# RemoteSensingTools/vSmartMOM.jl

Hardware: AMD Instinct MI355X
Metric: spectral-points/s (whole node) for rt_run, O2-A band (higher is better)
Workload: dtype f64; 1 GPU; C2: O2-A 759-770 nm, nStokes=3, Nquad=20 (N=60), 40 layers, 10000 spectral points/GPU, m=0..2, Rayleigh+synthetic O2 absorption, Lambertian 0.15; ranks=1, collective_backend=none (1 rank), N=60, layers=40, points_per_gpu=10000, fourier_moments=3

## Files before the change

### include/vsmartmom_hip.h

```cpp
#ifndef VSMARTMOM_HIP_H
#define VSMARTMOM_HIP_H

#include <stddef.h>
#include <stdint.h>

#ifdef __cplusplus
extern "C" {
#endif

typedef enum vsm_status {
  VSM_OK = 0,
  VSM_ERR_INVALID_ARG = 1,
  VSM_ERR_UNSUPPORTED = 2,
  VSM_ERR_HIP = 3,
  VSM_ERR_NO_DEVICE = 4
} vsm_status;

typedef enum vsm_iface {
  VSM_IFACE_00 = 0,
  VSM_IFACE_01 = 1,
  VSM_IFACE_10 = 2,
  VSM_IFACE_11 = 3
} vsm_iface;

// ... 310 lines not shown
                              const vsm_composite_f64* comp, const vsm_added_f64* added_scratch, void* stream);
int vsm_layer_forward_mix_f32(const vsm_quad_f32* q, int S, int m, int ndoubl, const float* dtau, const float* varpi,
                              const float* tau_sum, const float* F0, int ncomp, const float* Zpp_comp, const float* Zmp_comp,
                              const float* fcomp, float* z_scratch, int toa, const vsm_composite_f32* comp,
                              const vsm_added_f32* added_scratch, void* stream);
int vsm_mix_Z_f64(int N, int S, int ncomp, const double* Zpp_comp, const double* Zmp_comp, const double* fcomp, double* Zpp,
                  double* Zmp, void* stream);
int vsm_mix_Z_f32(int N, int S, int ncomp, const float* Zpp_comp, const float* Zmp_comp, const float* fcomp, float* Zpp,
                  float* Zmp, void* stream);
int vsm_mix_Z_moments_f64(int N, int S, int ncomp, int nm, const double* const* Zpp_comp_h, const double* const* Zmp_comp_h, int single,
                          const double* fcomp, double* Zpp, double* Zmp, void* stream);
int vsm_mix_Z_moments_f32(int N, int S, int ncomp, int nm, const float* const* Zpp_comp_h, const float* const* Zmp_comp_h, int single,
                          const float* fcomp, float* Zpp, float* Zmp, void* stream);

typedef struct vsm_run vsm_run;
enum { VSM_RUN_SOURCES_ONLY = 1, VSM_RUN_ZW_TAIL = 2 };
int vsm_run_supported(int N, int n_stokes, int coupling);
size_t vsm_run_workspace_bytes(int N, int n_stokes, int S, int nm, const int* coupling_h);
int vsm_run_supported_f32(int N, int n_stokes, int coupling);
size_t vsm_run_workspace_bytes_f32(int N, int n_stokes, int S, int nm, const int* coupling_h);
int vsm_run_create_f64(const vsm_quad_f64* q, int S, int nm, const int* m_h, const int* coupling_h, void* workspace,
                       size_t workspace_bytes, vsm_run** run);
int vsm_run_create_f32(const vsm_quad_f32* q, int S, int nm, const int* m_h, const int* coupling_h, void* workspace,
                       size_t workspace_bytes, vsm_run** run);
int vsm_run_create_ex_f64(const vsm_quad_f64* q, int S, int nm, const int* m_h, const int* coupling_h, void* workspace,
                          size_t workspace_bytes, unsigned flags, vsm_run** run);
int vsm_run_create_ex_f32(const vsm_quad_f32* q, int S, int nm, const int* m_h, const int* coupling_h, void* workspace,
                          size_t workspace_bytes, unsigned flags, vsm_run** run);
int vsm_run_layer_f64(vsm_run* run, int ndoubl, const double* dtau, const double* varpi, const double* tau_sum,
                      const double* F0, int ncomp, const double* const* Zpp, const double* const* Zmp, long long z_stride,
                      const double* fcomp, int toa, const int* layer_coupling_h, void* stream);
int vsm_run_layer_f32(vsm_run* run, int ndoubl, const float* dtau, const float* varpi, const float* tau_sum,
                      const float* F0, int ncomp, const float* const* Zpp, const float* const* Zmp, long long z_stride,
                      const float* fcomp, int toa, const int* layer_coupling_h, void* stream);
int vsm_run_export_f64(vsm_run* run, const vsm_composite_f64* comps, void* stream);
int vsm_run_export_f32(vsm_run* run, const vsm_composite_f32* comps, void* stream);
int vsm_run_import_f64(vsm_run* run, const vsm_composite_f64* comps, void* stream);
int vsm_run_import_f32(vsm_run* run, const vsm_composite_f32* comps, void* stream);
int vsm_run_zw_tail(vsm_run* run);
int vsm_run_destroy(vsm_run* run);
int vsm_stokes_coupling_f64(int N, int n_stokes, int nblocks, const double* Zpp, const double* Zmp, int* mask_d, void* stream);
int vsm_stokes_coupling_f32(int N, int n_stokes, int nblocks, const float* Zpp, const float* Zmp, int* mask_d, void* stream);

typedef struct vsm_added_rs_f64 {
  double *ier_mp, *iet_pp, *ier_pm, *iet_mm;
  double *ieJ0_p, *ieJ0_m;
  int K;
  int reserved;
} vsm_added_rs_f64;
typedef struct vsm_added_rs_f32 {
  float *ier_mp, *iet_pp, *ier_pm, *iet_mm;
  float *ieJ0_p, *ieJ0_m;
  int K;
  int reserved;
// ... 82 lines not shown
```

### vsmartmom.jl_amd/_lib.py

```python
from __future__ import annotations

import ctypes as C
import os

_HERE = os.path.dirname(os.path.abspath(__file__))
LIB_PATH = os.environ.get("VSM_LIB_PATH") or os.path.join(_HERE, "lib", "libvsmartmom_hip.so")


class VSMError(RuntimeError):
    pass


class vsm_quad_f64(C.Structure):
    _fields_ = [("mu", C.c_void_p), ("wt", C.c_void_p), ("N", C.c_int), ("n_stokes", C.c_int),
                ("i_mu0", C.c_int), ("mu0", C.c_double)]


class vsm_quad_f32(C.Structure):
    _fields_ = [("mu", C.c_void_p), ("wt", C.c_void_p), ("N", C.c_int), ("n_stokes", C.c_int),
                ("i_mu0", C.c_int), ("mu0", C.c_float)]


class vsm_added(C.Structure):
    _fields_ = [("r_mp", C.c_void_p), ("t_pp", C.c_void_p), ("r_pm", C.c_void_p), ("t_mm", C.c_void_p),
# ... 105 lines not shown
    "vsm_elemental_inelastic_rrs_{T}": (_I, [_P, _I, _I, _I, _P, _P, _P, _P, _P, _P]),
    "vsm_doubling_inelastic_rrs_{T}": (_I, [_I, _I, _I, _I, _P, _P, _P, _P, _P, _P]),
    "vsm_interaction_inelastic_rrs_{T}": (_I, [_I, _I, _I, _P, _P, _P, _P, _P, _P, _P]),
    "vsm_copy_added_to_composite_ie_{T}": (_I, [_I, _I, _P, _P, _P]),
    "vsm_postprocess_vza_ie_{T}": (_I, [_I, _I, _I, _I, _I, _P, _P, _P, _P, _P, _P, _P]),
    "vsm_run_supported": (_I, [_I, _I, _I]),
    "vsm_run_workspace_bytes": (_SZ, [_I, _I, _I, _I, _P]),
    "vsm_run_supported_f32": (_I, [_I, _I, _I]),
    "vsm_run_workspace_bytes_f32": (_SZ, [_I, _I, _I, _I, _P]),
    "vsm_run_create_{T}": (_I, [_P, _I, _I, _P, _P, _P, _SZ, _P]),
    "vsm_run_create_ex_{T}": (_I, [_P, _I, _I, _P, _P, _P, _SZ, C.c_uint, _P]),
    "vsm_run_layer_{T}": (_I, [_P, _I, _P, _P, _P, _P, _I, _P, _P, _LL, _P, _I, _P, _P]),
    "vsm_run_export_{T}": (_I, [_P, _P, _P]),
    "vsm_run_import_{T}": (_I, [_P, _P, _P]),
    "vsm_run_zw_tail": (_I, [_P]),
    "vsm_run_destroy": (_I, [_P]),
    "vsm_stokes_coupling_{T}": (_I, [_I, _I, _I, _P, _P, _P, _P]),
    "vsm_level_radiance_work_elems": (_SZ, [_I, _I]),
    "vsm_level_radiance_{T}": (_I, [_I, _I, _I, _I, _P, _P, _P, _P, _P, _LL, _P, _P, _P, _P, _P, _P, _P]),
    "vsm_level_radiance_oplevel_{T}": (_I, [_I, _I, _I, _I, _P, _P, _P, _P, _P, _LL, _P, _P, _P, _P, _P, _P, _P]),
    "vsm_test_lds_mm_{T}": (_I, [_I, _I, _P, _P, _P, _P]),
    "vsm_test_lds_inv_{T}": (_I, [_I, _I, _P, _P, _I, _P, _P]),
    "vsm_test_poison_lds": (_I, [_P]),
}


def exported_symbols():
    out = []
    for name in _SIGS:
        if "{T}" in name:
# ... 90 lines not shown
```

### vsmartmom.jl_amd/core_rt.py

```python
from __future__ import annotations

import ctypes as C
import dataclasses
import math
import os
from dataclasses import dataclass
from typing import List, Optional

import numpy as np
import torch

from . import _lib
from . import host_model as H
from .architectures import GPU, CPU, architecture, array_type, devi, synchronize_if_gpu, to_host

IFACE = {"00": 0, "01": 1, "10": 2, "11": 3}
MOMENT_BATCH = 4
MOMENT_BATCH_MAX = 24
MOMENT_BATCHING = True
THERMAL_FUSION = True
NATIVE_RUN = True
NATIVE_SOURCES_ONLY = True
NATIVE_ZW_TAIL = True
NATIVE_DROPIN = True
REFERENCE_ORDER = False


def _require_gpu(arch):
    if not isinstance(arch, GPU):
        raise _lib.VSMError("vsmartmom.jl_amd provides the MI355X path only; architecture %r has no compute path here "
                            "(no CPU fallback by design)" % (arch,))
    if not torch.cuda.is_available():
        raise _lib.VSMError("no MI355X visible to HIP (torch.cuda.is_available() is False)")
    if arch.device_index != torch.cuda.current_device():
        raise _lib.VSMError("architecture GPU(%d) is not the current HIP device (%d): one process per GPU -- call "
                            "torch.cuda.set_device(%d) first" % (arch.device_index, torch.cuda.current_device(),
                                                                 arch.device_index))

# ... 470 lines not shown

def _native_open(comp: CompositeLayer, dq: DeviceQuad, m: int, mask: int, import_arrays: bool) -> bool:
    L = _lib.lib()
    N, ns, S = comp.N, dq.n_stokes, comp.nSpec
    if not run_supported(comp.dtype, N, ns, mask):
        return False
    marr, carr = (C.c_int * 1)(int(m)), (C.c_int * 1)(int(mask))
    nbytes = run_workspace_bytes(comp.dtype, N, ns, S, 1, carr)
    ws = comp._native_ws
    if ws is None or ws.numel() * 8 < nbytes:
        ws = comp._native_ws = _lib.poison(torch.empty(max(nbytes // 8, 2), dtype=torch.float64, device=comp._arr["R_mp"].device))
    q = dq.cstruct()
    comp._native_q = (q, dq)
    run = C.c_void_p()
    flags = 1 if (comp._sources_only and NATIVE_SOURCES_ONLY) else 0
    _lib.call("vsm_run_create_ex", comp.dtype, C.byref(q), S, 1, marr, carr, _ptr(ws), nbytes, flags, C.byref(run))
    if import_arrays:
        try:
            cc = (_lib.vsm_composite * 1)(comp._cstruct_raw())
            _lib.call("vsm_run_import", comp.dtype, run, cc, _stream_ptr())
        except Exception:
            L.vsm_run_destroy(run)
            raise
    comp._native = NativeSlot(run, int(m), int(mask), stokes_groups(ns, mask))
    return True


def _rt_kernel_native(comp: CompositeLayer, props: DeviceLayerOptics, tau_sum, m: int, dq: DeviceQuad, iz: int, F0, dtau,
                      ndoubl: int) -> bool:
    N, ns, S = comp.N, dq.n_stokes, comp.nSpec
# ... 352 lines not shown
                return set()
        return {i for i, mom in enumerate(self.moments) if run_supported(self.dt, self.N, self.pol.n, int(self.coupling[mom["m"]]))}

    def _run_layers_native(self, group, comps, sources_only: bool = True, export_at=None):
        L = _lib.lib()
        nm, N, S, ns = len(group), self.N, self.S, self.pol.n
        marr = (C.c_int * nm)(*[int(mom["m"]) for mom in group])
        carr = (C.c_int * nm)(*[int(self.coupling[mom["m"]]) for mom in group])
        nbytes = run_workspace_bytes(self.dt, N, ns, S, nm, carr)
        ws = getattr(self, "_native_ws", None)
        if ws is None or ws.numel() * 8 < nbytes:
            ws = self._native_ws = _lib.poison(torch.empty(max(nbytes // 8, 2), dtype=torch.float64, device=self.dev))
        q = self.dq.cstruct()
        run = C.c_void_p()
        flags = 1 if (sources_only and NATIVE_SOURCES_ONLY) else 0
        _lib.call("vsm_run_create_ex", self.dt, C.byref(q), S, nm, marr, carr, _ptr(ws), nbytes, flags, C.byref(run))
        try:
            if NATIVE_ZW_TAIL and not torch.cuda.is_current_stream_capturing():
                _lib.check(L.vsm_run_zw_tail(run))
            for iz in range(self.Nz):
                ly0 = group[0]["layers"][iz]
                props = [mom["layers"][iz]["props"] for mom in group]
                p0 = props[0]
                zpp = (C.c_void_p * nm)(*[p.Zpp.data_ptr() for p in props])
                zmp = (C.c_void_p * nm)(*[p.Zmp.data_ptr() for p in props])
                ncomp = 0 if p0.fcomp is None else int(p0.fcomp.shape[1])
                lc = (C.c_int * nm)(*[self._layer_coupling(mom["m"], iz) for mom in group])
                run_layer_native_(run, nm, int(ly0["nd"]), ly0["dtau"], p0.varpi, ly0["tau_sum"], self.F0, ncomp, zpp, zmp,
                                  0 if ncomp else p0.z_stride, p0.fcomp, iz == 0, lc, self.dt)
                if export_at and (iz + 1) in export_at:
# ... 149 lines not shown
```

### vsmartmom.jl_amd/csrc/vsm_api.hip

```cpp
#include <map>
#include <mutex>
#include <set>
#include <utility>
#include <vector>
#include <stdlib.h>
#include <string.h>

#include "build_id.h"
#include "vsm_internal.h"

namespace vsm {

static thread_local char g_err[512] = "";

void set_error(const char* fmt, ...) {
  va_list ap;
  va_start(ap, fmt);
  vsnprintf(g_err, sizeof(g_err), fmt, ap);
  va_end(ap);
}
int hip_fail(hipError_t e, const char* what) {
  set_error("HIP error %d (%s) in %s", (int)e, hipGetErrorString(e), what);
  return VSM_ERR_HIP;
}
// ... 17 lines not shown
    return slot < o.slot;
  }
};
struct scratch_buf {
  void* ptr = nullptr;
  size_t sz = 0;
};
struct retired_buf {
  int dev;
  void* ptr;
  hipEvent_t ev;
};
std::mutex g_scratch_mu;
std::map<scratch_key, scratch_buf> g_scratch;
std::vector<retired_buf> g_retired;

void reap_retired(int dev, bool wait) {
  for (size_t i = 0; i < g_retired.size();) {
    retired_buf& r = g_retired[i];
    if (r.dev == dev && (wait ? hipEventSynchronize(r.ev) == hipSuccess : hipEventQuery(r.ev) == hipSuccess)) {
      (void)hipEventDestroy(r.ev);
      (void)hipFree(r.ptr);
      g_retired[i] = g_retired.back();
      g_retired.pop_back();
    } else {
      ++i;
    }
  }
}
}
// ... 31 lines not shown
    e = hipEventCreateWithFlags(&ev, hipEventDisableTiming);
    if (e == hipSuccess) e = hipEventRecord(ev, st);
    if (e != hipSuccess) {
      if (ev) (void)hipEventDestroy(ev);
      (void)hipFree(p);
      hip_fail(e, "hipEventRecord(scratch retire)");
      return nullptr;
    }
    g_retired.push_back(retired_buf{dev, b.ptr, ev});
  }
  b.ptr = p;
  b.sz = want;
  return p;
}

int release_scratch() {
  int dev = 0;
  hipError_t e = hipGetDevice(&dev);
  if (e != hipSuccess) return hip_fail(e, "hipGetDevice(release_scratch)");
  if ((e = hipDeviceSynchronize()) != hipSuccess) return hip_fail(e, "hipDeviceSynchronize(release_scratch)");
  std::lock_guard<std::mutex> lk(g_scratch_mu);
  reap_retired(dev, true);
  for (auto it = g_scratch.begin(); it != g_scratch.end();) {
    if (it->first.dev == dev) {
      if (it->second.ptr) (void)hipFree(it->second.ptr);
      it = g_scratch.erase(it);
    } else {
      ++it;
    }
  }
  return VSM_OK;
}

namespace {
std::mutex g_attr_mu;
std::set<std::pair<int, const void*>> g_attr_done;
std::mutex g_cu_mu;
std::map<int, int> g_cu;
}

namespace {
// ... 896 lines not shown
```

### vsmartmom.jl_amd/csrc/vsm_internal.h

```cpp
#pragma once
#include "vsm_common.h"

namespace vsm {

template <typename T>
struct quad {
  const T* mu;
  const T* wt;
  int N;
  int n_stokes;
  int i_mu0;
  T mu0;
};
template <typename T>
struct added {
  T *r_mp, *t_pp, *r_pm, *t_mm, *j0_p, *j0_m;
  long long mat_stride;
  int d_symmetric;
};
template <typename T>
struct composite {
  T *R_mp, *R_pm, *T_pp, *T_mm, *J0_p, *J0_m;
};

// ... 227 lines not shown
template <typename ST>
int strip128_doubling(int N, int n_stokes, int S, int ndoubl, ST* expk, const added<ST>& a, hipStream_t st);
template <typename ST>
int strip128_interaction11(int N, int S, const composite<ST>& c, const added<ST>& a, hipStream_t st);
inline bool strip128_f32_supported(int N) { return N > 96 && N <= 128; }

bool strip128_lin_dbl_supported(int N);
template <typename ST>
int strip128_doubling_lin(int N, int S, int P, int nd, int ns, ST* expk, ST* ekl, const added<ST>& a, const added_lin<ST>& al,
                          hipStream_t st);
template <typename ST>
int strip128_interaction11_lin(int N, int S, const composite<ST>& c, const composite_lin<ST>& cl, const added<ST>& a,
                               const added_lin<ST>& al, hipStream_t st);

void* scratch(size_t bytes, int slot, hipStream_t st);
int* device_status();
int release_scratch();
int ensure_dyn_lds(const void* kern, size_t bytes, const char* what);
int cu_count();

}
```

### vsmartmom.jl_amd/csrc/vsm_native.hip

```cpp
#include <stdlib.h>

#include <vector>

#include "vsm_native_dev.h"
#include "vsm_native_run.h"

#ifndef VSM_NATIVE_PARK_RT
#define VSM_NATIVE_PARK_RT 3
#endif

namespace vsm {

struct nlayer_comps {
  double* c[NSUB_MAX];
};

namespace {

template <int RT, int KS, int KZ = KS>
__device__ __forceinline__ void ned_body(nsmem<RT, (4 * KS + 2 > 16 * RT)>& sm, npos<RT>& p, int n, int gsz, unsigned uvmask, int ndoubl,
                                         const double* __restrict__ img, nstrip<RT>& r_s, nstrip<RT>& t_s, int* status) {
  using G = ngeo<RT>;
  constexpr unsigned dP = 0, dQ = G::AF * 8;
  double* jp = sm.vec[0];
// ... 1412 lines not shown
    bool zero = true;
    for (int a = 0; a < ns; ++a) zero = zero && w[(size_t)node * ns + a] == ST(0);
    if (!zero) break;
    ++z;
  }
  if (z == nq) z = 0;
  for (nat_sub& sb : run->subs) sb.kz = ((nq - z) * sb.gsz + 3) / 4;
  run->flags |= VSM_RUN_ZW_TAIL;
  return VSM_OK;
}

template <typename ST, typename Q>
static int run_create(const Q* q, int S, int nm, const int* m, const int* coupling, void* workspace, size_t workspace_bytes,
                      unsigned flags, vsm_run** run_out) {
  VSM_REQUIRE(q && q->mu && q->wt && run_out && m, "vsm_run_create: null argument");
  VSM_REQUIRE((flags & ~(unsigned)(VSM_RUN_SOURCES_ONLY | VSM_RUN_ZW_TAIL)) == 0, "vsm_run_create_ex: unknown flags 0x%x", flags);
  VSM_REQUIRE(S >= 0 && nm >= 1 && nm <= NSUB_MAX, "vsm_run_create: bad S = %d / nm = %d (at most %d moments per run)", S, nm,
              NSUB_MAX);
  vsm_run* run = new vsm_run;
  run->mu = q->mu;
  run->wt = q->wt;
  run->N = q->N;
  run->ns = q->n_stokes;
  run->i_mu0 = q->i_mu0;
  run->mu0 = (double)q->mu0;
  run->elem_size = (int)sizeof(ST);
  run->S = S;
  run->nm = nm;
  run->flags = sizeof(ST) == 8 ? flags : 0u;
  run->m.assign(m, m + nm);
  size_t total = 0;
  const int rc = plan_subs(sizeof(ST) == 4, q->N, q->n_stokes, nm, m, coupling, run->subs, (size_t)S, total);
  if (rc) {
    delete run;
    return rc;
  }
  if (total * sizeof(ST) > workspace_bytes || (total && !workspace) || ((size_t)workspace & 15)) {
    set_error("vsm_run_create: workspace of %zu bytes (16-byte aligned) required, got %zu", total * sizeof(ST), workspace_bytes);
    delete run;
    return VSM_ERR_INVALID_ARG;
  }
  if (run->flags & VSM_RUN_ZW_TAIL) {
    const int rc2 = zw_tail<ST>(run);
    if (rc2) {
// ... 10 lines not shown
    for (auto& cl : run->classes) {
      const nat_sub& h = run->subs[cl[0]];
      if (h.n == sb.n && h.gsz == sb.gsz && h.uvmask == sb.uvmask && (int)cl.size() < NSUB_MAX) {
        cl.push_back((int)i);
        placed = true;
        break;
      }
    }
    if (!placed) run->classes.push_back(std::vector<int>{(int)i});
  }
  *run_out = run;
  return VSM_OK;
}

template <typename ST>
static int run_layer(vsm_run* run, int ndoubl, const ST* dtau, const ST* varpi, const ST* tau_sum, const ST* F0, int ncomp,
                     const ST* const* Zpp, const ST* const* Zmp, long long z_stride, const ST* fcomp, int toa,
                     const int* layer_coupling, void* stream) {
  VSM_REQUIRE(run && dtau && varpi && tau_sum && F0 && Zpp && Zmp, "vsm_run_layer: null argument");
  VSM_REQUIRE(run->elem_size == (int)sizeof(ST), "vsm_run_layer: the run was created for %d-byte arrays", run->elem_size);
  VSM_REQUIRE(ndoubl >= 0 && ndoubl < 60 && ncomp >= 0 && ncomp <= 4 && (ncomp == 0 || fcomp), "vsm_run_layer: bad ndoubl / component mix");
  ++run->layers;
  if (run->S == 0) return VSM_OK;
  hipStream_t st = as_stream(stream);
  int* status = device_status();
  if (!status) return VSM_ERR_HIP;
  const quad<ST> q = run_quad<ST>(run);
  auto trivial = [&](const nat_sub& sb) {
    if (!layer_coupling || layer_coupling[sb.im] < 0) return false;
    for (int a = 0; a < sb.gsz; ++a)
      for (int b = 0; b < sb.gsz; ++b)
        if ((layer_coupling[sb.im] >> (4 * sb.g[a] + sb.g[b])) & 1) return false;
    return true;
  };
  {
    nguard_args<ST> ga;
    for (int k = 0; k < NSUB_MAX; ++k) {
      const int im = k < run->nm ? k : 0;
      VSM_REQUIRE(Zpp[im] && Zmp[im], "vsm_run_layer: null Z of moment %d", im);
      ga.zp[k] = Zpp[im];
      ga.zm[k] = Zmp[im];
      ga.allowed[k] = 0;
    }
    for (const nat_sub& sb : run->subs) {
      if (trivial(sb)) continue;
      for (int a = 0; a < sb.gsz; ++a)
        for (int b = 0; b < sb.gsz; ++b) ga.allowed[sb.im] |= 1u << (4 * sb.g[a] + sb.g[b]);
    }
    const int nmat = ncomp ? ncomp : (z_stride ? run->S : 1);
    hipLaunchKernelGGL((k_coupling_guard<ST>), dim3(nmat, run->nm), dim3(256), 0, st, run->N, run->ns,
                       ncomp ? (long long)run->N * run->N : z_stride, ga, status);
    VSM_LAUNCH_CHECK("k_coupling_guard");
  }
  if constexpr (sizeof(ST) == 4) {
    return native32_run_layer(run, ndoubl, dtau, varpi, tau_sum, F0, ncomp, Zpp, Zmp, z_stride, fcomp, toa, layer_coupling, status, st);
  } else {
  double* const ws = static_cast<double*>(run->ws);
  const int src = (run->flags & VSM_RUN_SOURCES_ONLY) ? 1 : 0;
  size_t pre_total = 0;
  for (const nat_sub& sb : run->subs)
    if (!trivial(sb)) pre_total += pre_stride_rt(sb.rt) * (size_t)run->S;
  double* pre = nullptr;
  if (pre_total) {
    pre = static_cast<double*>(scratch(pre_total * sizeof(double), 3, st));
    if (!pre) return VSM_ERR_HIP;
  }
  size_t off = 0;
  for (const auto& cl : run->classes) {
    const nat_sub& h = run->subs[cl[0]];
    std::vector<int> act, triv[3];
    for (int i : cl) {
      if (!trivial(run->subs[i])) {
        act.push_back(i);
        run->pure_diag[i] = 0;
      } else if (toa) {
        triv[1].push_back(i);
        run->pure_diag[i] = 1;
      } else {
        triv[run->pure_diag[i] ? 2 : 0].push_back(i);
      }
    }
    for (int mode = 0; mode < 3; ++mode) {
      if (triv[mode].empty()) continue;
      ndiag_args da;
      const int nt = (int)triv[mode].size();
      for (int k = 0; k < NSUB_MAX; ++k) {
        const nat_sub& sb = run->subs[triv[mode][k < nt ? k : 0]];
        da.comp[k] = ws + sb.comp_off;
        da.gsz[k] = sb.gsz;
        da.g0[k] = sb.g[0] | (sb.g[1] << 4) | (sb.g[2] << 8) | (sb.g[3] << 12);
      }
      hipLaunchKernelGGL((k_native_diag_layer<ST>), dim3(run->S, nt), dim3(256), 0, st, q, h.rt, h.n, ldexp(1.0, ndoubl), mode, src,
                         dtau, da);
      VSM_LAUNCH_CHECK("k_native_diag_layer");
    }
    const int nsub = (int)act.size();
    if (!nsub) continue;
    npre_args<ST> pa;
    nlayer_comps lc;
    for (int k = 0; k < NSUB_MAX; ++k) {
      const nat_sub& sb = run->subs[act[k < nsub ? k : 0]];
      pa.s[k].m = sb.m;
      pa.s[k].gsz = sb.gsz;
      for (int a = 0; a < 4; ++a) pa.s[k].g[a] = sb.g[a];
      VSM_REQUIRE(Zpp[sb.im] && Zmp[sb.im], "vsm_run_layer: null Z of moment %d", sb.im);
      pa.s[k].z = zsrc<ST>{Zpp[sb.im], Zmp[sb.im], ncomp ? 0 : z_stride, ncomp, fcomp};
      lc.c[k] = ws + sb.comp_off;
    }
    double* pre_cl = pre + off;
    off += pre_stride_rt(h.rt) * (size_t)run->S * nsub;
    switch (h.rt) {
      case 1: launch_pre<1, ST>(ncomp > 0, q, run->S, nsub, h.n, ndoubl, dtau, varpi, tau_sum, F0, pa, pre_cl, st); break;
      case 2: launch_pre<2, ST>(ncomp > 0, q, run->S, nsub, h.n, ndoubl, dtau, varpi, tau_sum, F0, pa, pre_cl, st); break;
      case 3: launch_pre<3, ST>(ncomp > 0, q, run->S, nsub, h.n, ndoubl, dtau, varpi, tau_sum, F0, pa, pre_cl, st); break;
      case 4: launch_pre<4, ST>(ncomp > 0, q, run->S, nsub, h.n, ndoubl, dtau, varpi, tau_sum, F0, pa, pre_cl, st); break;
      case 5: launch_pre<5, ST>(ncomp > 0, q, run->S, nsub, h.n, ndoubl, dtau, varpi, tau_sum, F0, pa, pre_cl, st); break;
      default: launch_pre<6, ST>(ncomp > 0, q, run->S, nsub, h.n, ndoubl, dtau, varpi, tau_sum, F0, pa, pre_cl, st); break;
    }
    VSM_LAUNCH_CHECK("k_elemental_native");
    const int rc = launch_layer_native(h.ks, h.ks - h.kz, run->S, nsub, h.n, h.uvmask, h.gsz, ndoubl, toa, src, pre_cl, lc, status, st);
    if (rc) return rc;
  }
  return VSM_OK;
  }
}

template <typename ST, typename CS, bool IMPORT>
static int run_convert(vsm_run* run, const CS* comps, void* stream) {
  VSM_REQUIRE(run && comps, "vsm_run_export / import: null argument");
  VSM_REQUIRE(run->elem_size == (int)sizeof(ST), "vsm_run_export / import: the run was created for %d-byte arrays", run->elem_size);
  if (run->S == 0) return VSM_OK;
  if (IMPORT) {
    run->pure_diag.assign(run->subs.size(), 0);
    run->flags &= ~(unsigned)VSM_RUN_ZW_TAIL;
    for (nat_sub& sb : run->subs) sb.kz = sb.ks;
  }
  for (int im = 0; im < run->nm; ++im) {
    const CS& c = comps[im];
    VSM_REQUIRE(c.R_mp && c.R_pm && c.T_pp && c.T_mm && c.J0_p && c.J0_m, "vsm_run_export / import: null composite array (moment %d)", im);
// ... 69 lines not shown
int vsm_run_create_ex_f64(const vsm_quad_f64* q, int S, int nm, const int* m, const int* coupling, void* workspace,
                          size_t workspace_bytes, unsigned flags, vsm_run** run_out) {
  return run_create<double>(q, S, nm, m, coupling, workspace, workspace_bytes, flags, run_out);
}
int vsm_run_create_ex_f32(const vsm_quad_f32* q, int S, int nm, const int* m, const int* coupling, void* workspace,
                          size_t workspace_bytes, unsigned flags, vsm_run** run_out) {
  return run_create<float>(q, S, nm, m, coupling, workspace, workspace_bytes, flags, run_out);
}

int vsm_run_zw_tail(vsm_run* run) {
  VSM_REQUIRE(run, "vsm_run_zw_tail: null argument");
  VSM_REQUIRE(run->layers == 0, "vsm_run_zw_tail: the run has taken layer steps already");
  return run->elem_size == 8 ? zw_tail<double>(run) : VSM_OK;
}

int vsm_run_destroy(vsm_run* run) {
  delete run;
  return VSM_OK;
}

int vsm_run_layer_f64(vsm_run* run, int ndoubl, const double* dtau, const double* varpi, const double* tau_sum, const double* F0,
                      int ncomp, const double* const* Zpp, const double* const* Zmp, long long z_stride, const double* fcomp,
                      int toa, const int* layer_coupling, void* stream) {
  return run_layer<double>(run, ndoubl, dtau, varpi, tau_sum, F0, ncomp, Zpp, Zmp, z_stride, fcomp, toa, layer_coupling, stream);
}
int vsm_run_layer_f32(vsm_run* run, int ndoubl, const float* dtau, const float* varpi, const float* tau_sum, const float* F0,
                      int ncomp, const float* const* Zpp, const float* const* Zmp, long long z_stride, const float* fcomp,
                      int toa, const int* layer_coupling, void* stream) {
  return run_layer<float>(run, ndoubl, dtau, varpi, tau_sum, F0, ncomp, Zpp, Zmp, z_stride, fcomp, toa, layer_coupling, stream);
}
// ... 25 lines not shown
```

### vsmartmom.jl_amd/csrc/vsm_native32.hip

```cpp
#include <stdlib.h>

#include <vector>

#include "vsm_native32_dev.h"
#include "vsm_native_run.h"

#ifndef VSM_N32_PARK_RT
#define VSM_N32_PARK_RT 5
#endif

namespace vsm {

struct n32layer_comps {
  float* c[NSUB_MAX];
};

namespace {

template <int RT, int KS>
__device__ __forceinline__ void n32ed_body(n32smem<RT, (4 * KS + 2 > 16 * RT)>& sm, n32pos<RT>& p, int n, int gsz, unsigned uvmask,
                                           int ndoubl, const float* __restrict__ img, n32strip<RT>& r_s, n32strip<RT>& t_s,
                                           int* status) {
  using G = n32geo<RT>;
  constexpr unsigned dP = 0, dQ = G::AF * 4;
// ... 694 lines not shown
                         const float* tau_sum, const float* F0, const n32pre_args& a, float* pre, hipStream_t st) {
  const dim3 grid(S, nsub), block(64 * RT);
  if (mix)
    hipLaunchKernelGGL((k_elemental_native32<RT, true>), grid, block, 0, st, q, n, ndoubl, dtau, varpi, tau_sum, F0, a, pre);
  else
    hipLaunchKernelGGL((k_elemental_native32<RT, false>), grid, block, 0, st, q, n, ndoubl, dtau, varpi, tau_sum, F0, a, pre);
}

}

int native32_rt_of(int n) { return native32_rt_of_ks((n + 3) / 4); }
size_t native32_comp_stride(int rt) { return (size_t)4 * (16 * rt) * (16 * rt) + 2 * 16 * rt; }

int native32_run_layer(vsm_run* run, int ndoubl, const float* dtau, const float* varpi, const float* tau_sum, const float* F0, int ncomp,
                       const float* const* Zpp, const float* const* Zmp, long long z_stride, const float* fcomp, int toa,
                       const int* layer_coupling, int* status, hipStream_t st) {
  const quad<float> q{static_cast<const float*>(run->mu), static_cast<const float*>(run->wt), run->N, run->ns, run->i_mu0, (float)run->mu0};
  float* ws = static_cast<float*>(run->ws);
  auto trivial = [&](const nat_sub& sb) {
    if (!layer_coupling || layer_coupling[sb.im] < 0) return false;
    for (int a = 0; a < sb.gsz; ++a)
      for (int b = 0; b < sb.gsz; ++b)
        if ((layer_coupling[sb.im] >> (4 * sb.g[a] + sb.g[b])) & 1) return false;
    return true;
  };
  size_t pre_total = 0;
  for (const nat_sub& sb : run->subs)
    if (!trivial(sb)) pre_total += pre32_stride_rt(sb.rt) * (size_t)run->S;
  float* pre = nullptr;
  if (pre_total) {
    pre = static_cast<float*>(scratch(pre_total * sizeof(float), 3, st));
    if (!pre) return VSM_ERR_HIP;
  }
  size_t off = 0;
  for (const auto& cl : run->classes) {
    const nat_sub& h = run->subs[cl[0]];
    std::vector<int> act, triv[3];
    for (int i : cl) {
      if (!trivial(run->subs[i])) {
        act.push_back(i);
        run->pure_diag[i] = 0;
      } else if (toa) {
        triv[1].push_back(i);
        run->pure_diag[i] = 1;
      } else {
        triv[run->pure_diag[i] ? 2 : 0].push_back(i);
      }
    }
    for (int mode = 0; mode < 3; ++mode) {
      if (triv[mode].empty()) continue;
      n32diag_args da;
      const int nt = (int)triv[mode].size();
      for (int k = 0; k < NSUB_MAX; ++k) {
        const nat_sub& sb = run->subs[triv[mode][k < nt ? k : 0]];
        da.comp[k] = ws + sb.comp_off;
        da.gsz[k] = sb.gsz;
        da.g0[k] = sb.g[0] | (sb.g[1] << 4) | (sb.g[2] << 8) | (sb.g[3] << 12);
      }
      hipLaunchKernelGGL(k_native32_diag_layer, dim3(run->S, nt), dim3(256), 0, st, q, h.rt, h.n, (float)ldexp(1.0, ndoubl), mode, dtau,
                         da);
      VSM_LAUNCH_CHECK("k_native32_diag_layer");
    }
    const int nsub = (int)act.size();
    if (!nsub) continue;
    n32pre_args pa;
    n32layer_comps lc;
    for (int k = 0; k < NSUB_MAX; ++k) {
      const nat_sub& sb = run->subs[act[k < nsub ? k : 0]];
      pa.s[k].m = sb.m;
      pa.s[k].gsz = sb.gsz;
      for (int a = 0; a < 4; ++a) pa.s[k].g[a] = sb.g[a];
      VSM_REQUIRE(Zpp[sb.im] && Zmp[sb.im], "vsm_run_layer: null Z of moment %d", sb.im);
      pa.s[k].z = zsrc<float>{Zpp[sb.im], Zmp[sb.im], ncomp ? 0 : z_stride, ncomp, fcomp};
      lc.c[k] = ws + sb.comp_off;
    }
    float* pre_cl = pre + off;
    off += pre32_stride_rt(h.rt) * (size_t)run->S * nsub;
    switch (h.rt) {
      case 1: launch_pre32<1>(ncomp > 0, q, run->S, nsub, h.n, ndoubl, dtau, varpi, tau_sum, F0, pa, pre_cl, st); break;
      case 2: launch_pre32<2>(ncomp > 0, q, run->S, nsub, h.n, ndoubl, dtau, varpi, tau_sum, F0, pa, pre_cl, st); break;
      case 3: launch_pre32<3>(ncomp > 0, q, run->S, nsub, h.n, ndoubl, dtau, varpi, tau_sum, F0, pa, pre_cl, st); break;
      case 4: launch_pre32<4>(ncomp > 0, q, run->S, nsub, h.n, ndoubl, dtau, varpi, tau_sum, F0, pa, pre_cl, st); break;
      case 5: launch_pre32<5>(ncomp > 0, q, run->S, nsub, h.n, ndoubl, dtau, varpi, tau_sum, F0, pa, pre_cl, st); break;
      case 6: launch_pre32<6>(ncomp > 0, q, run->S, nsub, h.n, ndoubl, dtau, varpi, tau_sum, F0, pa, pre_cl, st); break;
      case 7: launch_pre32<7>(ncomp > 0, q, run->S, nsub, h.n, ndoubl, dtau, varpi, tau_sum, F0, pa, pre_cl, st); break;
      default: launch_pre32<8>(ncomp > 0, q, run->S, nsub, h.n, ndoubl, dtau, varpi, tau_sum, F0, pa, pre_cl, st); break;
    }
    VSM_LAUNCH_CHECK("k_elemental_native32");
    const int rc = launch_layer_native32(h.ks, run->S, nsub, h.n, h.uvmask, h.gsz, ndoubl, toa, pre_cl, lc, status, st);
    if (rc) return rc;
  }
  return VSM_OK;
}

int native32_convert(vsm_run* run, int im, const composite<float>& c, bool import, hipStream_t st) {
  n32group_map gm;
  gm.ngroups = 0;
  for (int a = 0; a < 4; ++a) {
    gm.grp_of[a] = gm.pos_in[a] = 0;
    gm.gsz[a] = gm.rt[a] = 1;
    gm.n[a] = 0;
    gm.base[a] = nullptr;
  }
  for (const nat_sub& sb : run->subs) {
// ... 23 lines not shown
```

### vsmartmom.jl_amd/csrc/vsm_native_run.h

```cpp
#pragma once
#include <vector>

#include "vsm_internal.h"

namespace vsm {

constexpr int NSUB_MAX = VSM_MM_MAX;

struct nat_sub {
  int im;
  int m;
  int gsz, g[4];
  unsigned uvmask;
  int n, rt, ks;
  int kz;
  size_t comp_off;
};

}

struct vsm_run {
  const void *mu, *wt;
  int N, ns, i_mu0;
  double mu0;
  int elem_size;
  int S, nm;
  unsigned flags;
  std::vector<int> m;
  std::vector<vsm::nat_sub> subs;
  std::vector<std::vector<int>> classes;
  void* ws;
  size_t ws_elems;
  int layers = 0;
  std::vector<char> pure_diag;
};

namespace vsm {

constexpr int NATIVE_MAX_ROWS = 96;
constexpr int NATIVE32_MAX_ROWS = 128;
int native32_rt_of(int n);
size_t native32_comp_stride(int rt);
int native32_run_layer(vsm_run* run, int ndoubl, const float* dtau, const float* varpi, const float* tau_sum, const float* F0,
                       int ncomp, const float* const* Zpp, const float* const* Zmp, long long z_stride, const float* fcomp, int toa,
                       const int* layer_coupling, int* status, hipStream_t st);
int native32_convert(vsm_run* run, int im, const composite<float>& c, bool import, hipStream_t st);

}
```

Baseline: 26040 spectral-points/s.

## Overlap independent Stokes-coupling classes on an auxiliary stream per layer

Per layer, the heaviest class of sub-problems stays on the caller's stream and all other non-trivial classes are issued on a cached auxiliary stream. Fork and join events link the two streams so the classes can run concurrently instead of back to back. A flag and a Python toggle bring back the serial order, and overlap is skipped during graph capture. The cost is two extra event records and waits per layer, and the side-stream classes share one stream, so they still run serially among themselves.

```diff
diff --git a/include/vsmartmom_hip.h b/include/vsmartmom_hip.h
--- a/include/vsmartmom_hip.h
+++ b/include/vsmartmom_hip.h
@@ -348,7 +348,7 @@
                           const float* fcomp, float* Zpp, float* Zmp, void* stream);
 
 typedef struct vsm_run vsm_run;
-enum { VSM_RUN_SOURCES_ONLY = 1, VSM_RUN_ZW_TAIL = 2 };
+enum { VSM_RUN_SOURCES_ONLY = 1, VSM_RUN_ZW_TAIL = 2, VSM_RUN_SERIAL_CLASSES = 8 };
 int vsm_run_supported(int N, int n_stokes, int coupling);
 size_t vsm_run_workspace_bytes(int N, int n_stokes, int S, int nm, const int* coupling_h);
 int vsm_run_supported_f32(int N, int n_stokes, int coupling);
@@ -372,6 +372,7 @@
 int vsm_run_import_f64(vsm_run* run, const vsm_composite_f64* comps, void* stream);
 int vsm_run_import_f32(vsm_run* run, const vsm_composite_f32* comps, void* stream);
 int vsm_run_zw_tail(vsm_run* run);
+unsigned vsm_run_flags(const vsm_run* run);
 int vsm_run_destroy(vsm_run* run);
 int vsm_stokes_coupling_f64(int N, int n_stokes, int nblocks, const double* Zpp, const double* Zmp, int* mask_d, void* stream);
 int vsm_stokes_coupling_f32(int N, int n_stokes, int nblocks, const float* Zpp, const float* Zmp, int* mask_d, void* stream);
diff --git a/vsmartmom.jl_amd/_lib.py b/vsmartmom.jl_amd/_lib.py
--- a/vsmartmom.jl_amd/_lib.py
+++ b/vsmartmom.jl_amd/_lib.py
@@ -143,6 +143,7 @@
     "vsm_run_export_{T}": (_I, [_P, _P, _P]),
     "vsm_run_import_{T}": (_I, [_P, _P, _P]),
     "vsm_run_zw_tail": (_I, [_P]),
+    "vsm_run_flags": (C.c_uint, [_P]),
     "vsm_run_destroy": (_I, [_P]),
     "vsm_stokes_coupling_{T}": (_I, [_I, _I, _I, _P, _P, _P, _P]),
     "vsm_level_radiance_work_elems": (_SZ, [_I, _I]),
diff --git a/vsmartmom.jl_amd/core_rt.py b/vsmartmom.jl_amd/core_rt.py
--- a/vsmartmom.jl_amd/core_rt.py
+++ b/vsmartmom.jl_amd/core_rt.py
@@ -22,6 +22,7 @@
 NATIVE_RUN = True
 NATIVE_SOURCES_ONLY = True
 NATIVE_ZW_TAIL = True
+NATIVE_OVERLAP = True
 NATIVE_DROPIN = True
 REFERENCE_ORDER = False
 
@@ -522,6 +523,7 @@
     comp._native_q = (q, dq)
     run = C.c_void_p()
     flags = 1 if (comp._sources_only and NATIVE_SOURCES_ONLY) else 0
+    flags |= 0 if NATIVE_OVERLAP else 8
     _lib.call("vsm_run_create_ex", comp.dtype, C.byref(q), S, 1, marr, carr, _ptr(ws), nbytes, flags, C.byref(run))
     if import_arrays:
         try:
@@ -904,6 +906,7 @@
         q = self.dq.cstruct()
         run = C.c_void_p()
         flags = 1 if (sources_only and NATIVE_SOURCES_ONLY) else 0
+        flags |= 0 if NATIVE_OVERLAP else 8
         _lib.call("vsm_run_create_ex", self.dt, C.byref(q), S, nm, marr, carr, _ptr(ws), nbytes, flags, C.byref(run))
         try:
             if NATIVE_ZW_TAIL and not torch.cuda.is_current_stream_capturing():
diff --git a/vsmartmom.jl_amd/csrc/vsm_api.hip b/vsmartmom.jl_amd/csrc/vsm_api.hip
--- a/vsmartmom.jl_amd/csrc/vsm_api.hip
+++ b/vsmartmom.jl_amd/csrc/vsm_api.hip
@@ -55,6 +55,7 @@
 std::mutex g_scratch_mu;
 std::map<scratch_key, scratch_buf> g_scratch;
 std::vector<retired_buf> g_retired;
+std::map<scratch_key, side_chain> g_side;
 
 void reap_retired(int dev, bool wait) {
   for (size_t i = 0; i < g_retired.size();) {
@@ -116,6 +117,34 @@
   return p;
 }
 
+const side_chain* side_chain_of(hipStream_t st) {
+  int dev = 0;
+  hipError_t e = hipGetDevice(&dev);
+  if (e != hipSuccess) {
+    hip_fail(e, "hipGetDevice(side_chain_of)");
+    return nullptr;
+  }
+  if (st == hipStreamPerThread) {
+    set_error("hipStreamPerThread is not accepted by the entry points that use library scratch: pass the thread's own stream handle");
+    return nullptr;
+  }
+  std::lock_guard<std::mutex> lk(g_scratch_mu);
+  auto it = g_side.find(scratch_key{dev, st, 0});
+  if (it != g_side.end()) return &it->second;
+  side_chain c{nullptr, nullptr, nullptr};
+  e = hipStreamCreateWithFlags(&c.aux, hipStreamNonBlocking);
+  if (e == hipSuccess) e = hipEventCreateWithFlags(&c.fork, hipEventDisableTiming);
+  if (e == hipSuccess) e = hipEventCreateWithFlags(&c.join, hipEventDisableTiming);
+  if (e != hipSuccess) {
+    if (c.join) (void)hipEventDestroy(c.join);
+    if (c.fork) (void)hipEventDestroy(c.fork);
+    if (c.aux) (void)hipStreamDestroy(c.aux);
+    hip_fail(e, "hipStreamCreate / hipEventCreate(side_chain_of)");
+    return nullptr;
+  }
+  return &(g_side[scratch_key{dev, st, 0}] = c);
+}
+
 int release_scratch() {
   int dev = 0;
   hipError_t e = hipGetDevice(&dev);
@@ -127,6 +156,16 @@
     if (it->first.dev == dev) {
       if (it->second.ptr) (void)hipFree(it->second.ptr);
       it = g_scratch.erase(it);
+    } else {
+      ++it;
+    }
+  }
+  for (auto it = g_side.begin(); it != g_side.end();) {
+    if (it->first.dev == dev) {
+      (void)hipEventDestroy(it->second.join);
+      (void)hipEventDestroy(it->second.fork);
+      (void)hipStreamDestroy(it->second.aux);
+      it = g_side.erase(it);
     } else {
       ++it;
     }
diff --git a/vsmartmom.jl_amd/csrc/vsm_internal.h b/vsmartmom.jl_amd/csrc/vsm_internal.h
--- a/vsmartmom.jl_amd/csrc/vsm_internal.h
+++ b/vsmartmom.jl_amd/csrc/vsm_internal.h
@@ -265,6 +265,11 @@
                                const added_lin<ST>& al, hipStream_t st);
 
 void* scratch(size_t bytes, int slot, hipStream_t st);
+struct side_chain {
+  hipStream_t aux;
+  hipEvent_t fork, join;
+};
+const side_chain* side_chain_of(hipStream_t st);
 int* device_status();
 int release_scratch();
 int ensure_dyn_lds(const void* kern, size_t bytes, const char* what);
diff --git a/vsmartmom.jl_amd/csrc/vsm_native.hip b/vsmartmom.jl_amd/csrc/vsm_native.hip
--- a/vsmartmom.jl_amd/csrc/vsm_native.hip
+++ b/vsmartmom.jl_amd/csrc/vsm_native.hip
@@ -1450,7 +1450,8 @@
 static int run_create(const Q* q, int S, int nm, const int* m, const int* coupling, void* workspace, size_t workspace_bytes,
                       unsigned flags, vsm_run** run_out) {
   VSM_REQUIRE(q && q->mu && q->wt && run_out && m, "vsm_run_create: null argument");
-  VSM_REQUIRE((flags & ~(unsigned)(VSM_RUN_SOURCES_ONLY | VSM_RUN_ZW_TAIL)) == 0, "vsm_run_create_ex: unknown flags 0x%x", flags);
+  VSM_REQUIRE((flags & ~(unsigned)(VSM_RUN_SOURCES_ONLY | VSM_RUN_ZW_TAIL | VSM_RUN_SERIAL_CLASSES)) == 0,
+              "vsm_run_create_ex: unknown flags 0x%x", flags);
   VSM_REQUIRE(S >= 0 && nm >= 1 && nm <= NSUB_MAX, "vsm_run_create: bad S = %d / nm = %d (at most %d moments per run)", S, nm,
               NSUB_MAX);
   vsm_run* run = new vsm_run;
@@ -1463,7 +1464,7 @@
   run->elem_size = (int)sizeof(ST);
   run->S = S;
   run->nm = nm;
-  run->flags = sizeof(ST) == 8 ? flags : 0u;
+  run->flags = sizeof(ST) == 8 ? flags : flags & (unsigned)VSM_RUN_SERIAL_CLASSES;
   run->m.assign(m, m + nm);
   size_t total = 0;
   const int rc = plan_subs(sizeof(ST) == 4, q->N, q->n_stokes, nm, m, coupling, run->subs, (size_t)S, total);
@@ -1504,47 +1505,15 @@
 }
 
 template <typename ST>
-static int run_layer(vsm_run* run, int ndoubl, const ST* dtau, const ST* varpi, const ST* tau_sum, const ST* F0, int ncomp,
-                     const ST* const* Zpp, const ST* const* Zmp, long long z_stride, const ST* fcomp, int toa,
-                     const int* layer_coupling, void* stream) {
-  VSM_REQUIRE(run && dtau && varpi && tau_sum && F0 && Zpp && Zmp, "vsm_run_layer: null argument");
-  VSM_REQUIRE(run->elem_size == (int)sizeof(ST), "vsm_run_layer: the run was created for %d-byte arrays", run->elem_size);
-  VSM_REQUIRE(ndoubl >= 0 && ndoubl < 60 && ncomp >= 0 && ncomp <= 4 && (ncomp == 0 || fcomp), "vsm_run_layer: bad ndoubl / component mix");
-  ++run->layers;
-  if (run->S == 0) return VSM_OK;
-  hipStream_t st = as_stream(stream);
-  int* status = device_status();
-  if (!status) return VSM_ERR_HIP;
+static int run_layer_classes(vsm_run* run, int ndoubl, const ST* dtau, const ST* varpi, const ST* tau_sum, const ST* F0, int ncomp,
+                             const ST* const* Zpp, const ST* const* Zmp, long long z_stride, const ST* fcomp, int toa,
+                             const int* layer_coupling, int* status, hipStream_t st, const hipStream_t* cst) {
+  if constexpr (sizeof(ST) == 4) {
+    return native32_run_layer(run, ndoubl, dtau, varpi, tau_sum, F0, ncomp, Zpp, Zmp, z_stride, fcomp, toa, layer_coupling, status, st,
+                              cst);
+  } else {
   const quad<ST> q = run_quad<ST>(run);
-  auto trivial = [&](const nat_sub& sb) {
-    if (!layer_coupling || layer_coupling[sb.im] < 0) return false;
-    for (int a = 0; a < sb.gsz; ++a)
-      for (int b = 0; b < sb.gsz; ++b)
-        if ((layer_coupling[sb.im] >> (4 * sb.g[a] + sb.g[b])) & 1) return false;
-    return true;
-  };
-  {
-    nguard_args<ST> ga;
-    for (int k = 0; k < NSUB_MAX; ++k) {
-      const int im = k < run->nm ? k : 0;
-      VSM_REQUIRE(Zpp[im] && Zmp[im], "vsm_run_layer: null Z of moment %d", im);
-      ga.zp[k] = Zpp[im];
-      ga.zm[k] = Zmp[im];
-      ga.allowed[k] = 0;
-    }
-    for (const nat_sub& sb : run->subs) {
-      if (trivial(sb)) continue;
-      for (int a = 0; a < sb.gsz; ++a)
-        for (int b = 0; b < sb.gsz; ++b) ga.allowed[sb.im] |= 1u << (4 * sb.g[a] + sb.g[b]);
-    }
-    const int nmat = ncomp ? ncomp : (z_stride ? run->S : 1);
-    hipLaunchKernelGGL((k_coupling_guard<ST>), dim3(nmat, run->nm), dim3(256), 0, st, run->N, run->ns,
-                       ncomp ? (long long)run->N * run->N : z_stride, ga, status);
-    VSM_LAUNCH_CHECK("k_coupling_guard");
-  }
-  if constexpr (sizeof(ST) == 4) {
-    return native32_run_layer(run, ndoubl, dtau, varpi, tau_sum, F0, ncomp, Zpp, Zmp, z_stride, fcomp, toa, layer_coupling, status, st);
-  } else {
+  auto trivial = [&](const nat_sub& sb) { return layer_trivial(sb, layer_coupling); };
   double* const ws = static_cast<double*>(run->ws);
   const int src = (run->flags & VSM_RUN_SOURCES_ONLY) ? 1 : 0;
   size_t pre_total = 0;
@@ -1556,7 +1525,9 @@
     if (!pre) return VSM_ERR_HIP;
   }
   size_t off = 0;
-  for (const auto& cl : run->classes) {
+  for (size_t ci = 0; ci < run->classes.size(); ++ci) {
+    const std::vector<int>& cl = run->classes[ci];
+    const hipStream_t cs = cst[ci];
     const nat_sub& h = run->subs[cl[0]];
     std::vector<int> act, triv[3];
     for (int i : cl) {
@@ -1580,7 +1551,7 @@
         da.gsz[k] = sb.gsz;
         da.g0[k] = sb.g[0] | (sb.g[1] << 4) | (sb.g[2] << 8) | (sb.g[3] << 12);
       }
-      hipLaunchKernelGGL((k_native_diag_layer<ST>), dim3(run->S, nt), dim3(256), 0, st, q, h.rt, h.n, ldexp(1.0, ndoubl), mode, src,
+      hipLaunchKernelGGL((k_native_diag_layer<ST>), dim3(run->S, nt), dim3(256), 0, cs, q, h.rt, h.n, ldexp(1.0, ndoubl), mode, src,
                          dtau, da);
       VSM_LAUNCH_CHECK("k_native_diag_layer");
     }
@@ -1600,19 +1571,89 @@
     double* pre_cl = pre + off;
     off += pre_stride_rt(h.rt) * (size_t)run->S * nsub;
     switch (h.rt) {
-      case 1: launch_pre<1, ST>(ncomp > 0, q, run->S, nsub, h.n, ndoubl, dtau, varpi, tau_sum, F0, pa, pre_cl, st); break;
-      case 2: launch_pre<2, ST>(ncomp > 0, q, run->S, nsub, h.n, ndoubl, dtau, varpi, tau_sum, F0, pa, pre_cl, st); break;
-      case 3: launch_pre<3, ST>(ncomp > 0, q, run->S, nsub, h.n, ndoubl, dtau, varpi, tau_sum, F0, pa, pre_cl, st); break;
-      case 4: launch_pre<4, ST>(ncomp > 0, q, run->S, nsub, h.n, ndoubl, dtau, varpi, tau_sum, F0, pa, pre_cl, st); break;
-      case 5: launch_pre<5, ST>(ncomp > 0, q, run->S, nsub, h.n, ndoubl, dtau, varpi, tau_sum, F0, pa, pre_cl, st); break;
-      default: launch_pre<6, ST>(ncomp > 0, q, run->S, nsub, h.n, ndoubl, dtau, varpi, tau_sum, F0, pa, pre_cl, st); break;
+      case 1: launch_pre<1, ST>(ncomp > 0, q, run->S, nsub, h.n, ndoubl, dtau, varpi, tau_sum, F0, pa, pre_cl, cs); break;
+      case 2: launch_pre<2, ST>(ncomp > 0, q, run->S, nsub, h.n, ndoubl, dtau, varpi, tau_sum, F0, pa, pre_cl, cs); break;
+      case 3: launch_pre<3, ST>(ncomp > 0, q, run->S, nsub, h.n, ndoubl, dtau, varpi, tau_sum, F0, pa, pre_cl, cs); break;
+      case 4: launch_pre<4, ST>(ncomp > 0, q, run->S, nsub, h.n, ndoubl, dtau, varpi, tau_sum, F0, pa, pre_cl, cs); break;
+      case 5: launch_pre<5, ST>(ncomp > 0, q, run->S, nsub, h.n, ndoubl, dtau, varpi, tau_sum, F0, pa, pre_cl, cs); break;
+      default: launch_pre<6, ST>(ncomp > 0, q, run->S, nsub, h.n, ndoubl, dtau, varpi, tau_sum, F0, pa, pre_cl, cs); break;
     }
     VSM_LAUNCH_CHECK("k_elemental_native");
-    const int rc = launch_layer_native(h.ks, h.ks - h.kz, run->S, nsub, h.n, h.uvmask, h.gsz, ndoubl, toa, src, pre_cl, lc, status, st);
+    const int rc = launch_layer_native(h.ks, h.ks - h.kz, run->S, nsub, h.n, h.uvmask, h.gsz, ndoubl, toa, src, pre_cl, lc, status, cs);
     if (rc) return rc;
   }
   return VSM_OK;
   }
+}
+
+template <typename ST>
+static int run_layer(vsm_run* run, int ndoubl, const ST* dtau, const ST* varpi, const ST* tau_sum, const ST* F0, int ncomp,
+                     const ST* const* Zpp, const ST* const* Zmp, long long z_stride, const ST* fcomp, int toa,
+                     const int* layer_coupling, void* stream) {
+  VSM_REQUIRE(run && dtau && varpi && tau_sum && F0 && Zpp && Zmp, "vsm_run_layer: null argument");
+  VSM_REQUIRE(run->elem_size == (int)sizeof(ST), "vsm_run_layer: the run was created for %d-byte arrays", run->elem_size);
+  VSM_REQUIRE(ndoubl >= 0 && ndoubl < 60 && ncomp >= 0 && ncomp <= 4 && (ncomp == 0 || fcomp), "vsm_run_layer: bad ndoubl / component mix");
+  ++run->layers;
+  if (run->S == 0) return VSM_OK;
+  hipStream_t st = as_stream(stream);
+  int* status = device_status();
+  if (!status) return VSM_ERR_HIP;
+  auto trivial = [&](const nat_sub& sb) { return layer_trivial(sb, layer_coupling); };
+  {
+    nguard_args<ST> ga;
+    for (int k = 0; k < NSUB_MAX; ++k) {
+      const int im = k < run->nm ? k : 0;
+      VSM_REQUIRE(Zpp[im] && Zmp[im], "vsm_run_layer: null Z of moment %d", im);
+      ga.zp[k] = Zpp[im];
+      ga.zm[k] = Zmp[im];
+      ga.allowed[k] = 0;
+    }
+    for (const nat_sub& sb : run->subs) {
+      if (trivial(sb)) continue;
+      for (int a = 0; a < sb.gsz; ++a)
+        for (int b = 0; b < sb.gsz; ++b) ga.allowed[sb.im] |= 1u << (4 * sb.g[a] + sb.g[b]);
+    }
+    const int nmat = ncomp ? ncomp : (z_stride ? run->S : 1);
+    hipLaunchKernelGGL((k_coupling_guard<ST>), dim3(nmat, run->nm), dim3(256), 0, st, run->N, run->ns,
+                       ncomp ? (long long)run->N * run->N : z_stride, ga, status);
+    VSM_LAUNCH_CHECK("k_coupling_guard");
+  }
+  std::vector<hipStream_t> cst(run->classes.size(), st);
+  const side_chain* sc = nullptr;
+  if (!(run->flags & VSM_RUN_SERIAL_CLASSES)) {
+    int nbusy = 0, big = -1;
+    double wbig = 0.0;
+    for (size_t ci = 0; ci < run->classes.size(); ++ci) {
+      double w = 0.0;
+      for (int i : run->classes[ci])
+        if (!trivial(run->subs[i])) w += (double)run->subs[i].ks * run->subs[i].ks * run->subs[i].ks;
+      if (w > 0.0) ++nbusy;
+      if (w > wbig) {
+        wbig = w;
+        big = (int)ci;
+      }
+    }
+    hipStreamCaptureStatus cap = hipStreamCaptureStatusNone;
+    if (nbusy > 1 && hipStreamIsCapturing(st, &cap) != hipSuccess) {
+      (void)hipGetLastError();
+      cap = hipStreamCaptureStatusActive;
+    }
+    if (nbusy > 1 && cap == hipStreamCaptureStatusNone && st != hipStreamPerThread) {
+      sc = side_chain_of(st);
+      if (!sc) return VSM_ERR_HIP;
+      VSM_HIP(hipEventRecord(sc->fork, st));
+      VSM_HIP(hipStreamWaitEvent(sc->aux, sc->fork, 0));
+      for (size_t ci = 0; ci < cst.size(); ++ci)
+        if ((int)ci != big) cst[ci] = sc->aux;
+    }
+  }
+  const int rc = run_layer_classes<ST>(run, ndoubl, dtau, varpi, tau_sum, F0, ncomp, Zpp, Zmp, z_stride, fcomp, toa, layer_coupling,
+                                       status, st, cst.data());
+  if (sc) {
+    VSM_HIP(hipEventRecord(sc->join, sc->aux));
+    VSM_HIP(hipStreamWaitEvent(st, sc->join, 0));
+  }
+  return rc;
 }
 
 template <typename ST, typename CS, bool IMPORT>
@@ -1712,6 +1753,8 @@
   return run->elem_size == 8 ? zw_tail<double>(run) : VSM_OK;
 }
 
+unsigned vsm_run_flags(const vsm_run* run) { return run ? run->flags : 0u; }
+
 int vsm_run_destroy(vsm_run* run) {
   delete run;
   return VSM_OK;
diff --git a/vsmartmom.jl_amd/csrc/vsm_native32.hip b/vsmartmom.jl_amd/csrc/vsm_native32.hip
--- a/vsmartmom.jl_amd/csrc/vsm_native32.hip
+++ b/vsmartmom.jl_amd/csrc/vsm_native32.hip
@@ -732,16 +732,10 @@
 
 int native32_run_layer(vsm_run* run, int ndoubl, const float* dtau, const float* varpi, const float* tau_sum, const float* F0, int ncomp,
                        const float* const* Zpp, const float* const* Zmp, long long z_stride, const float* fcomp, int toa,
-                       const int* layer_coupling, int* status, hipStream_t st) {
+                       const int* layer_coupling, int* status, hipStream_t st, const hipStream_t* cst) {
   const quad<float> q{static_cast<const float*>(run->mu), static_cast<const float*>(run->wt), run->N, run->ns, run->i_mu0, (float)run->mu0};
   float* ws = static_cast<float*>(run->ws);
-  auto trivial = [&](const nat_sub& sb) {
-    if (!layer_coupling || layer_coupling[sb.im] < 0) return false;
-    for (int a = 0; a < sb.gsz; ++a)
-      for (int b = 0; b < sb.gsz; ++b)
-        if ((layer_coupling[sb.im] >> (4 * sb.g[a] + sb.g[b])) & 1) return false;
-    return true;
-  };
+  auto trivial = [&](const nat_sub& sb) { return layer_trivial(sb, layer_coupling); };
   size_t pre_total = 0;
   for (const nat_sub& sb : run->subs)
     if (!trivial(sb)) pre_total += pre32_stride_rt(sb.rt) * (size_t)run->S;
@@ -751,7 +745,9 @@
     if (!pre) return VSM_ERR_HIP;
   }
   size_t off = 0;
-  for (const auto& cl : run->classes) {
+  for (size_t ci = 0; ci < run->classes.size(); ++ci) {
+    const std::vector<int>& cl = run->classes[ci];
+    const hipStream_t cs = cst[ci];
     const nat_sub& h = run->subs[cl[0]];
     std::vector<int> act, triv[3];
     for (int i : cl) {
@@ -775,7 +771,7 @@
         da.gsz[k] = sb.gsz;
         da.g0[k] = sb.g[0] | (sb.g[1] << 4) | (sb.g[2] << 8) | (sb.g[3] << 12);
       }
-      hipLaunchKernelGGL(k_native32_diag_layer, dim3(run->S, nt), dim3(256), 0, st, q, h.rt, h.n, (float)ldexp(1.0, ndoubl), mode, dtau,
+      hipLaunchKernelGGL(k_native32_diag_layer, dim3(run->S, nt), dim3(256), 0, cs, q, h.rt, h.n, (float)ldexp(1.0, ndoubl), mode, dtau,
                          da);
       VSM_LAUNCH_CHECK("k_native32_diag_layer");
     }
@@ -795,17 +791,17 @@
     float* pre_cl = pre + off;
     off += pre32_stride_rt(h.rt) * (size_t)run->S * nsub;
     switch (h.rt) {
-      case 1: launch_pre32<1>(ncomp > 0, q, run->S, nsub, h.n, ndoubl, dtau, varpi, tau_sum, F0, pa, pre_cl, st); break;
-      case 2: launch_pre32<2>(ncomp > 0, q, run->S, nsub, h.n, ndoubl, dtau, varpi, tau_sum, F0, pa, pre_cl, st); break;
-      case 3: launch_pre32<3>(ncomp > 0, q, run->S, nsub, h.n, ndoubl, dtau, varpi, tau_sum, F0, pa, pre_cl, st); break;
-      case 4: launch_pre32<4>(ncomp > 0, q, run->S, nsub, h.n, ndoubl, dtau, varpi, tau_sum, F0, pa, pre_cl, st); break;
-      case 5: launch_pre32<5>(ncomp > 0, q, run->S, nsub, h.n, ndoubl, dtau, varpi, tau_sum, F0, pa, pre_cl, st); break;
-      case 6: launch_pre32<6>(ncomp > 0, q, run->S, nsub, h.n, ndoubl, dtau, varpi, tau_sum, F0, pa, pre_cl, st); break;
-      case 7: launch_pre32<7>(ncomp > 0, q, run->S, nsub, h.n, ndoubl, dtau, varpi, tau_sum, F0, pa, pre_cl, st); break;
-      default: launch_pre32<8>(ncomp > 0, q, run->S, nsub, h.n, ndoubl, dtau, varpi, tau_sum, F0, pa, pre_cl, st); break;
+      case 1: launch_pre32<1>(ncomp > 0, q, run->S, nsub, h.n, ndoubl, dtau, varpi, tau_sum, F0, pa, pre_cl, cs); break;
+      case 2: launch_pre32<2>(ncomp > 0, q, run->S, nsub, h.n, ndoubl, dtau, varpi, tau_sum, F0, pa, pre_cl, cs); break;
+      case 3: launch_pre32<3>(ncomp > 0, q, run->S, nsub, h.n, ndoubl, dtau, varpi, tau_sum, F0, pa, pre_cl, cs); break;
+      case 4: launch_pre32<4>(ncomp > 0, q, run->S, nsub, h.n, ndoubl, dtau, varpi, tau_sum, F0, pa, pre_cl, cs); break;
+      case 5: launch_pre32<5>(ncomp > 0, q, run->S, nsub, h.n, ndoubl, dtau, varpi, tau_sum, F0, pa, pre_cl, cs); break;
+      case 6: launch_pre32<6>(ncomp > 0, q, run->S, nsub, h.n, ndoubl, dtau, varpi, tau_sum, F0, pa, pre_cl, cs); break;
+      case 7: launch_pre32<7>(ncomp > 0, q, run->S, nsub, h.n, ndoubl, dtau, varpi, tau_sum, F0, pa, pre_cl, cs); break;
+      default: launch_pre32<8>(ncomp > 0, q, run->S, nsub, h.n, ndoubl, dtau, varpi, tau_sum, F0, pa, pre_cl, cs); break;
     }
     VSM_LAUNCH_CHECK("k_elemental_native32");
-    const int rc = launch_layer_native32(h.ks, run->S, nsub, h.n, h.uvmask, h.gsz, ndoubl, toa, pre_cl, lc, status, st);
+    const int rc = launch_layer_native32(h.ks, run->S, nsub, h.n, h.uvmask, h.gsz, ndoubl, toa, pre_cl, lc, status, cs);
     if (rc) return rc;
   }
   return VSM_OK;
diff --git a/vsmartmom.jl_amd/csrc/vsm_native_run.h b/vsmartmom.jl_amd/csrc/vsm_native_run.h
--- a/vsmartmom.jl_amd/csrc/vsm_native_run.h
+++ b/vsmartmom.jl_amd/csrc/vsm_native_run.h
@@ -16,6 +16,14 @@
   int kz;
   size_t comp_off;
 };
+
+inline bool layer_trivial(const nat_sub& sb, const int* layer_coupling) {
+  if (!layer_coupling || layer_coupling[sb.im] < 0) return false;
+  for (int a = 0; a < sb.gsz; ++a)
+    for (int b = 0; b < sb.gsz; ++b)
+      if ((layer_coupling[sb.im] >> (4 * sb.g[a] + sb.g[b])) & 1) return false;
+  return true;
+}
 
 }
 
@@ -43,7 +51,7 @@
 size_t native32_comp_stride(int rt);
 int native32_run_layer(vsm_run* run, int ndoubl, const float* dtau, const float* varpi, const float* tau_sum, const float* F0,
                        int ncomp, const float* const* Zpp, const float* const* Zmp, long long z_stride, const float* fcomp, int toa,
-                       const int* layer_coupling, int* status, hipStream_t st);
+                       const int* layer_coupling, int* status, hipStream_t st, const hipStream_t* cst);
 int native32_convert(vsm_run* run, int im, const composite<float>& c, bool import, hipStream_t st);
 
 }
```

Measured after the change: 26080 spectral-points/s (median of 6 runs). No clear change (+0.2%).
